# xiezheng-cs/PyTorch_Distributed_Template

Measured on AMD Instinct MI355X. Metric: images/sec (node) ResNet-18 DDP bs=1200/GPU at 1/2/4/8 MI355X, higher is better.
Workload: dtype bf16; 1 GPU; model=resnet18, global_batch=1200, parallelism=dp1, per_gpu_batch=1200, sync_bn=False, engine=native-hip, comm=none, grad_compress=none

## Files before the change

csrc/kernels/conv_fwd.h:

```cpp
#pragma once
#include <hip/hip_runtime.h>
#include <stdint.h>

#include "conv_geom.h"

namespace pdt {

constexpr int kStatSlots = 64;

void stat_rows_reduce_launch(const float* rows, int R, int CK, double* slots, hipStream_t s, int slots_ld = 0);


struct ConvFwdArgs : ConvGeom {
  const uint16_t* x;
  const uint16_t* w;
  uint16_t* y;
  const uint16_t* res;
  double* stats;
  int bnb;
  const uint16_t* bn_y1;
  const float* bn_coef1;
  const uint16_t* bn_y2;
  const float* bn_coef2;
  const uint8_t* bn_mask;
  int pair_skip;
  int res_phase = -1;
  int stage_out = 0;
  const float* pre_coef = nullptr;
  int ldy = 0, coef_ld = 0, stats_ld = 0;
  int nslice = 0;
  int64_t slice_wstride = 0;
  int srows_coff = 0;
};

void conv_fwd_launch(const ConvFwdArgs& a, int dtype, int bm, int bn, int bk, hipStream_t s);
int conv_fwd_m_tiles(int64_t M, int bm);

}
```

csrc/kernels/conv_fwd.hip:

```cpp
#include <cstdlib>

#include "../common.h"
#include "conv_fwd.h"
#include "conv_l1.h"

namespace pdt {

typedef __attribute__((address_space(3))) void lds_void;
typedef __attribute__((address_space(1))) void glb_void;

template <int CHUNKS>
PDT_DEVICE int swz(int row) { return (row >> 1) & (CHUNKS - 1); }

template <int DT, int EPI, int RES, int FN, int FM, int WN, int WM, int BN, int WAVES_M, int NW_, int SMEM = 0,
          bool PERM = false>
PDT_DEVICE void conv_epilogue(const ConvFwdArgs& a, f32x4_t (&acc)[FN][FM], int64_t m0, int n0, int tile_m, int wn,
                              int wm, int tid, int lane, char* smem) {
  using E = E16<DT>;
  const int fr = lane & 15, fq = lane >> 4;
  const int PQ = a.Pm * a.Qm;
  const FastDiv fd_pq{a.pq_mul, a.pq_shift}, fd_q{a.q_mul, a.q_shift};
  constexpr int KS = EPI == 0 ? 0 : (EPI == 4 ? 3 : 2);
  float sacc[FN][4][KS > 0 ? KS : 1];
#pragma unroll
  for (int i = 0; i < FN; ++i)
#pragma unroll
    for (int r = 0; r < 4; ++r)
#pragma unroll
      for (int k = 0; k < (KS > 0 ? KS : 1); ++k) sacc[i][r][k] = 0.f;

  constexpr int RED_BYTES = WAVES_M * BN * 3 * 4;
  float* cf = (float*)(smem + RED_BYTES);
  const int64_t LDY = a.ldy ? a.ldy : a.Kout;
  if constexpr (EPI >= 2) {
    const int CL = a.coef_ld ? a.coef_ld : a.Kout;
    for (int c = tid; c < BN; c += NW_ * 64) {
      const int n = n0 + c;
      cf[0 * BN + c] = a.bn_coef1[n];
      cf[1 * BN + c] = a.bn_coef1[CL + n];
      cf[2 * BN + c] = a.bn_coef1[2 * CL + n];
      cf[3 * BN + c] = a.bn_coef1[3 * CL + n];
      if constexpr (EPI == 4) {
        cf[4 * BN + c] = a.bn_coef2[2 * CL + n];
        cf[5 * BN + c] = a.bn_coef2[3 * CL + n];
      }
    }
    __syncthreads();
  }
  auto chan = [&](int i, int r) { return PERM ? (i >> 1) * 32 + 8 * fq + 4 * (i & 1) + r : i * 16 + 4 * fq + r; };
  static_assert(!PERM || FN % 2 == 0, "PERM pairs fragments");
  auto coef4 = [&](int q, int i) { return *(const float4*)(cf + q * BN + wn * WN + chan(i, 0)); };

  constexpr bool LY1 = EPI >= 2, LY2 = EPI == 4, LM = EPI == 3 || EPI == 4;
  static_assert(!LM || WN % 64 == 0, "bitmask epilogue needs 64-channel wave columns");
  constexpr int MW = LM ? WN / 64 : 1;
  constexpr int PER_J = FN * (2 * (RES != 0) + 2 * LY1 + 2 * LY2) + (LM ? 2 * MW : 0);
  constexpr int BUDGET = (FN * FM * 4 >= 128 ? 64 : 96) - (KS > 2 ? FN * 4 * (KS - 2) * 2 : 0);
  constexpr int JC = PER_J == 0 ? FM
                     : (8 * PER_J <= BUDGET && FM % 8 == 0) ? 8
                     : (4 * PER_J <= BUDGET && FM % 4 == 0) ? 4
                     : (2 * PER_J <= BUDGET && FM % 2 == 0) ? 2 : 1;
  static_assert(FM % JC == 0, "epilogue chunking");
  constexpr int BM_T = WAVES_M * WM;
  constexpr int SPITCH = BN * 2 + 16;
  constexpr int STG_OFF = 16384;
  constexpr bool FULL = SMEM >= STG_OFF + BM_T * SPITCH;
  constexpr bool PERGRP = !FULL && WAVES_M > 1 && EPI != 2 && SMEM >= STG_OFF + WM * SPITCH;
  constexpr bool CAN_STAGE = FULL || PERGRP;
  static_assert(!CAN_STAGE || RED_BYTES + 6 * BN * 4 <= STG_OFF, "epilogue LDS regions overlap");
  const bool stage = CAN_STAGE && a.stage_out;
  char* stg = smem + STG_OFF;
  const int srow0 = FULL ? wm * WM : 0;
  constexpr bool RC = RES == 2;
  const bool res_on = !RC || (int)blockIdx.y == a.res_phase;
  auto copy_rows = [&](int g) {
    constexpr int CPR = BN / 8;
    constexpr int SROWS = FULL ? BM_T : WM;
    for (int q = tid; q < SROWS * CPR; q += NW_ * 64) {
      const int row = q / CPR, ch = q - row * CPR;
      const int64_t m = m0 + (FULL ? 0 : g * WM) + row;
      if (m < a.M) {
        const int mm = (int)m;
        const int nimg = (int)fdiv((uint32_t)mm, fd_pq);
        const int rem = mm - nimg * PQ;
        const int i_ = (int)fdiv((uint32_t)rem, fd_q), j_ = rem - i_ * a.Qm;
        const int oh = i_ * a.ost_h + a.ooff_h, ow = j_ * a.ost_w + a.ooff_w;
        const int64_t ob = (((int64_t)nimg * a.OH + oh) * a.OW + ow) * LDY + n0 + ch * 8;
        *(uint4*)(a.y + ob) = *(const uint4*)(stg + row * SPITCH + ch * 16);
      }
    }
  };
  if constexpr (PERGRP) {
    if (stage)
      for (int g = 0; g < wm; ++g) {
        __syncthreads();
        copy_rows(g);
        __syncthreads();
      }
  }
#pragma unroll
  for (int jc = 0; jc < FM; jc += JC) {
    int64_t obase[JC];
    uint32_t rbase[RC ? JC : 1];
    bool valid[JC];
#pragma unroll
    for (int jj = 0; jj < JC; ++jj) {
      const int64_t m = m0 + wm * WM + (jc + jj) * 16 + fr;
      valid[jj] = m < a.M;
      const int mm = valid[jj] ? (int)m : 0;
      const int nimg = (int)fdiv((uint32_t)mm, fd_pq);
      const int rem = mm - nimg * PQ;
      const int i_ = (int)fdiv((uint32_t)rem, fd_q), j_ = rem - i_ * a.Qm;
      const int oh = i_ * a.ost_h + a.ooff_h, ow = j_ * a.ost_w + a.ooff_w;
      obase[jj] = (((int64_t)nimg * a.OH + oh) * a.OW + ow) * LDY;
      if constexpr (RC) rbase[jj] = (uint32_t)mm * (uint32_t)LDY;
    }
    uint2 p_res[RES ? JC : 1][RES ? FN : 1], p_y1[LY1 ? JC : 1][LY1 ? FN : 1], p_y2[LY2 ? JC : 1][LY2 ? FN : 1];
    uint64_t p_m[LM ? JC : 1][MW];
#pragma unroll
    for (int jj = 0; jj < JC; ++jj) {
      if constexpr (PERM) {
#pragma unroll
        for (int i = 0; i < FN; i += 2) {
          const int64_t o = obase[jj] + n0 + wn * WN + chan(i, 0);
          auto split = [&](uint2 (&dst)[FN], const uint4 v) {
            dst[i] = make_uint2(v.x, v.y);
            dst[i + 1] = make_uint2(v.z, v.w);
          };
          if constexpr (RES == 1) split(p_res[jj], *(const uint4*)(a.res + o));
          if constexpr (RC) split(p_res[jj], *(const uint4*)(a.res + rbase[jj] + (uint32_t)(n0 + wn * WN + chan(i, 0))));
          if constexpr (LY1) split(p_y1[jj], *(const uint4*)(a.bn_y1 + o));
          if constexpr (LY2) split(p_y2[jj], *(const uint4*)(a.bn_y2 + o));
        }
      } else {
#pragma unroll
        for (int i = 0; i < FN; ++i) {
          const int64_t o = obase[jj] + n0 + wn * WN + i * 16 + 4 * fq;
          if constexpr (RES == 1) p_res[jj][i] = *(const uint2*)(a.res + o);
          if constexpr (RC) p_res[jj][i] = *(const uint2*)(a.res + rbase[jj] + (uint32_t)(n0 + wn * WN + i * 16 + 4 * fq));
          if constexpr (LY1) p_y1[jj][i] = *(const uint2*)(a.bn_y1 + o);
          if constexpr (LY2) p_y2[jj][i] = *(const uint2*)(a.bn_y2 + o);
        }
      }
      if constexpr (LM) {
#pragma unroll
        for (int g = 0; g < MW; ++g)
          p_m[jj][g] = *(const uint64_t*)(a.bn_mask + ((obase[jj] + n0 + wn * WN + g * 64) >> 3));
      }
    }
#pragma unroll
    for (int jj = 0; jj < JC; ++jj) {
      if (!valid[jj]) continue;
      const int j = jc + jj;
      uint2 held = make_uint2(0u, 0u);
#pragma unroll
      for (int i = 0; i < FN; ++i) {
        const int n = n0 + wn * WN + chan(i, 0);
        const int64_t o = obase[jj] + n;
        float v[4] = {acc[i][j][0], acc[i][j][1], acc[i][j][2], acc[i][j][3]};
        if constexpr (RES) {
          uint2 rr = p_res[jj][i];
          if constexpr (RC) {
            rr.x = res_on ? rr.x : 0u;
            rr.y = res_on ? rr.y : 0u;
          }
          v[0] += E::to_f((uint16_t)(rr.x & 0xffff));
          v[1] += E::to_f((uint16_t)(rr.x >> 16));
          v[2] += E::to_f((uint16_t)(rr.y & 0xffff));
          v[3] += E::to_f((uint16_t)(rr.y >> 16));
        }
        float y1[4], y2[4];
        if constexpr (LY1) {
          const uint2 q1 = p_y1[jj][i];
          y1[0] = E::to_f((uint16_t)(q1.x & 0xffff)); y1[1] = E::to_f((uint16_t)(q1.x >> 16));
          y1[2] = E::to_f((uint16_t)(q1.y & 0xffff)); y1[3] = E::to_f((uint16_t)(q1.y >> 16));
          if constexpr (EPI == 2) {
            const float4 sc = coef4(0, i), sh = coef4(1, i);
            if (!(y1[0] * sc.x + sh.x > 0.f)) v[0] = 0.f;
            if (!(y1[1] * sc.y + sh.y > 0.f)) v[1] = 0.f;
            if (!(y1[2] * sc.z + sh.z > 0.f)) v[2] = 0.f;
            if (!(y1[3] * sc.w + sh.w > 0.f)) v[3] = 0.f;
          } else {
            const uint32_t mb = (uint32_t)(p_m[jj][chan(i, 0) >> 6] >> (chan(i, 0) & 63));
            if (!(mb & 1u)) v[0] = 0.f;
            if (!(mb & 2u)) v[1] = 0.f;
            if (!(mb & 4u)) v[2] = 0.f;
            if (!(mb & 8u)) v[3] = 0.f;
          }
        }
        if constexpr (LY2) {
          const uint2 q2 = p_y2[jj][i];
          y2[0] = E::to_f((uint16_t)(q2.x & 0xffff)); y2[1] = E::to_f((uint16_t)(q2.x >> 16));
          y2[2] = E::to_f((uint16_t)(q2.y & 0xffff)); y2[3] = E::to_f((uint16_t)(q2.y >> 16));
        }
        uint2 packed;
        packed.x = E::pack2(v[0], v[1]);
        packed.y = E::pack2(v[2], v[3]);
        const uint16_t ov[4] = {(uint16_t)packed.x, (uint16_t)(packed.x >> 16), (uint16_t)packed.y,
                                (uint16_t)(packed.y >> 16)};
        if (CAN_STAGE && stage) {
          if constexpr (PERM) {
            if (i & 1)
              *(uint4*)(stg + (srow0 + j * 16 + fr) * SPITCH + (wn * WN + chan(i, 0) - 4) * 2) =
                  make_uint4(held.x, held.y, packed.x, packed.y);
            else
              held = packed;
          } else {
            *(uint2*)(stg + (srow0 + j * 16 + fr) * SPITCH + (wn * WN + chan(i, 0)) * 2) = packed;
          }
        } else if constexpr (PERM) {
          if (i & 1)
            *(uint4*)(a.y + o - 4) = make_uint4(held.x, held.y, packed.x, packed.y);
          else
            held = packed;
        } else {
          *(uint2*)(a.y + o) = packed;
        }
        if constexpr (EPI == 1) {
#pragma unroll
          for (int r = 0; r < 4; ++r) {
            const float q = E::to_f(ov[r]);
            sacc[i][r][0] += q;
            sacc[i][r][1] += q * q;
          }
        } else if constexpr (EPI >= 2) {
          const float4 mu = coef4(2, i), is = coef4(3, i);
          const float m1[4] = {mu.x, mu.y, mu.z, mu.w}, i1[4] = {is.x, is.y, is.z, is.w};
#pragma unroll
          for (int r = 0; r < 4; ++r) {
            const float dz = E::to_f(ov[r]);
            sacc[i][r][0] += dz;
            sacc[i][r][1] += dz * (y1[r] - m1[r]) * i1[r];
          }
          if constexpr (EPI == 4) {
            const float4 mu2 = coef4(4, i), is2 = coef4(5, i);
            const float m2[4] = {mu2.x, mu2.y, mu2.z, mu2.w}, i2[4] = {is2.x, is2.y, is2.z, is2.w};
#pragma unroll
            for (int r = 0; r < 4; ++r) sacc[i][r][2] += E::to_f(ov[r]) * (y2[r] - m2[r]) * i2[r];
          }
        }
      }
    }
  }

  if constexpr (CAN_STAGE) {
    if (stage) {
      if constexpr (PERGRP) {
        for (int g = wm; g < WAVES_M; ++g) {
          __syncthreads();
          copy_rows(g);
          __syncthreads();
        }
      } else {
        __syncthreads();
        copy_rows(0);
      }
    }
  }

  if constexpr (KS > 0) {
    constexpr int KO = EPI == 4 ? 4 : 2;
#pragma unroll
    for (int i = 0; i < FN; ++i)
#pragma unroll
      for (int r = 0; r < 4; ++r)
#pragma unroll
        for (int k = 0; k < KS; ++k) sacc[i][r][k] = row16_sum(sacc[i][r][k]);
    float* red = (float*)smem;
    __syncthreads();
    if (fr == 15) {
#pragma unroll
      for (int i = 0; i < FN; ++i)
#pragma unroll
        for (int r = 0; r < 4; ++r) {
          const int nl = wn * WN + chan(i, r);
#pragma unroll
          for (int k = 0; k < KS; ++k) red[(wm * BN + nl) * KS + k] = sacc[i][r][k];
        }
    }
    __syncthreads();
    if (tid < BN) {
      float t[KS];
#pragma unroll
      for (int k = 0; k < KS; ++k) t[k] = 0.f;
#pragma unroll
      for (int w = 0; w < WAVES_M; ++w)
#pragma unroll
        for (int k = 0; k < KS; ++k) t[k] += red[(w * BN + tid) * KS + k];
      const int64_t row = (a.nphase > 0 ? (int64_t)blockIdx.y * a.srows_pp : 0) + tile_m;
// ... 21 lines not shown
template <int DT, int BM, int BN, int BK, int WAVES_N, int EPI, int RES, int STAGES, int NW>
__global__ __launch_bounds__(NW * 64, (STAGES * (BN + BM) * BK * 2 <= 81920 || NW == 8) ? 2 : 1)
void conv_fwd_kernel(ConvFwdArgs args) {
  ConvFwdArgs a = args;
  const uint16_t* wbase = args.w;
  if (args.nslice > 1) {
    const int sl = blockIdx.z;
    a.x += (int64_t)sl * a.Kout;
    a.y += (int64_t)sl * a.Kout;
    wbase += (int64_t)sl * args.slice_wstride;
    a.w = wbase;
    if (a.bn_y1 != nullptr) a.bn_y1 += (int64_t)sl * a.Kout;
    if (a.bn_coef1 != nullptr) a.bn_coef1 += sl * a.Kout;
    a.srows_coff = sl * a.Kout;
  }
  if (args.nphase > 0 && !select_phase(a, args, wbase, blockIdx.y)) {
    zero_stat_row<EPI, BN>(a, NW * 64);
    return;
  }
  using E = E16<DT>;
  typedef typename E::vec8 vec8;
  constexpr int WAVES_M = NW / WAVES_N;
  constexpr int WN = BN / WAVES_N;
  constexpr int WM = BM / WAVES_M;
  constexpr int FN = WN / 16, FM = WM / 16;
  constexpr int ROWB = BK * 2;
  constexpr int CHUNKS = ROWB / 16;
  constexpr int RPI = 1024 / ROWB;
  constexpr int A_INSTR = BN / RPI / NW;
  constexpr int B_INSTR = BM / RPI / NW;
  constexpr int A_BYTES = BN * ROWB;
  constexpr int STAGE = (BN + BM) * ROWB;
  static_assert(A_INSTR * RPI * NW == BN && B_INSTR * RPI * NW == BM, "tile/instr mismatch");
  __shared__ __attribute__((aligned(1024))) char smem[STAGES * STAGE];

  const int tid = threadIdx.x;
  const int lane = tid & 63;
  const int wave = __builtin_amdgcn_readfirstlane(tid >> 6);
  const int wn = wave % WAVES_N, wm = wave / WAVES_N;

  const int nwg = a.m_tiles * a.n_tiles;
  const int bid = xcd_remap(blockIdx.x, nwg);
  const int tile_m = bid / a.n_tiles, tile_n = bid % a.n_tiles;
  const int64_t m0 = (int64_t)tile_m * BM;
  const int n0 = tile_n * BN;

  const int PQ = a.Pm * a.Qm;
  const FastDiv fd_pq{a.pq_mul, a.pq_shift}, fd_q{a.q_mul, a.q_shift};
  const int TU = a.T * a.U;
  const int csteps = a.C / BK;
  const int ksteps = TU * csteps;

  const __amdgpu_buffer_rsrc_t rx = make_rsrc(a.x, (uint32_t)a.N * a.H * a.W * a.cs * 2u);
  const __amdgpu_buffer_rsrc_t rw = make_rsrc(a.w, (uint32_t)a.Kout * TU * a.C * 2u);

  const int lrow = lane / CHUNKS;
  const int pchunk = lane % CHUNKS;
  int brow_h[B_INSTR], brow_w[B_INSTR], brow_off[B_INSTR];
#pragma unroll
  for (int j = 0; j < B_INSTR; ++j) {
    const int row = (wave * B_INSTR + j) * RPI + lrow;
    const int64_t m = m0 + row;
    const int bch = pchunk ^ swz<CHUNKS>(row);
    if (m < a.M) {
      const int nimg = (int)fdiv((uint32_t)m, fd_pq);
      const int rem = (int)m - nimg * PQ;
      const int i = (int)fdiv((uint32_t)rem, fd_q), jj = rem - i * a.Qm;
      brow_h[j] = i * a.ist_h + a.ioff_h;
      brow_w[j] = jj * a.ist_w + a.ioff_w;
      const int pair = (CHUNKS == 8 && bch >= 4) ? a.pair_skip : 0;
      brow_off[j] = (((nimg * a.H + brow_h[j]) * a.W + brow_w[j]) * a.cs + bch * 8 + pair) * 2;
    } else {
      brow_h[j] = -(1 << 29);
      brow_w[j] = 0;
      brow_off[j] = 0;
    }
  }
  constexpr bool PERM = WN % 32 == 0;
  uint32_t arow_off[A_INSTR];
#pragma unroll
  for (int j = 0; j < A_INSTR; ++j) {
    const int row = (wave * A_INSTR + j) * RPI + lrow;
    const int lw = row % WN, fi = lw >> 4, fm = lw & 15;
    const int ch = PERM ? row - lw + (fi >> 1) * 32 + (fm >> 2) * 8 + (fi & 1) * 4 + (fm & 3) : row;
// ... 33 lines not shown
  const int fr = lane & 15, fq = lane >> 4;
  int a_off[FN], b_off[FM];
#pragma unroll
  for (int i = 0; i < FN; ++i) a_off[i] = (wn * WN + i * 16 + fr) * ROWB;
#pragma unroll
  for (int j = 0; j < FM; ++j) b_off[j] = A_BYTES + (wm * WM + j * 16 + fr) * ROWB;

  auto compute_stage = [&](const char* sb) {
#pragma unroll
    for (int kk = 0; kk < BK / 32; ++kk) {
      vec8 af[FN], bfr[FM];
#pragma unroll
      for (int i = 0; i < FN; ++i) {
        const int row = wn * WN + i * 16 + fr;
        const int ch = (kk * 4 + fq) ^ swz<CHUNKS>(row);
        af[i] = *(const vec8*)(sb + a_off[i] + ch * 16);
      }
#pragma unroll
      for (int j = 0; j < FM; ++j) {
        const int row = wm * WM + j * 16 + fr;
        const int ch = (kk * 4 + fq) ^ swz<CHUNKS>(row);
        bfr[j] = *(const vec8*)(sb + b_off[j] + ch * 16);
      }
#pragma unroll
      for (int i = 0; i < FN; ++i)
#pragma unroll
        for (int j = 0; j < FM; ++j) acc[i][j] = E::mfma16x16x32(af[i], bfr[j], acc[i][j]);
    }
  };

  if constexpr (STAGES == 2) {
    if (ksteps > 0) {
      stage_load(0);
      asm volatile("s_waitcnt vmcnt(0)" ::: "memory");
      __syncthreads();
      for (int ks = 0; ks < ksteps; ++ks) {
        const int cur = ks & 1;
        if (ks + 1 < ksteps) stage_load(cur ^ 1);
        compute_stage(smem + cur * STAGE);
        asm volatile("s_waitcnt vmcnt(0)" ::: "memory");
        __syncthreads();
      }
    }
  } else {
    constexpr int S = STAGES;
    constexpr int PER_STAGE = A_INSTR + B_INSTR;
    auto wait_ahead = [&](int ahead) {
      constexpr int W1 = PER_STAGE, W2 = 2 * PER_STAGE;
      if (ahead >= 2)
        __builtin_amdgcn_s_waitcnt((W2 & 0xF) | ((W2 >> 4) << 14) | (0x7 << 4) | (0xF << 8));
      else if (ahead == 1)
        __builtin_amdgcn_s_waitcnt((W1 & 0xF) | ((W1 >> 4) << 14) | (0x7 << 4) | (0xF << 8));
      else
        asm volatile("s_waitcnt vmcnt(0)" ::: "memory");
    };
    static_assert(S <= 4, "wait_ahead covers at most two stages in flight");
    if (ksteps > 0) {
#pragma unroll
      for (int p = 0; p < S - 1; ++p)
        if (p < ksteps) stage_load(p);
      int buf = 0;
      for (int ks = 0; ks < ksteps; ++ks) {
        const int ahead = min(S - 2, ksteps - 1 - ks);
        wait_ahead(ahead);
        __builtin_amdgcn_s_barrier();
        if (ks + S - 1 < ksteps) stage_load(buf == 0 ? S - 1 : buf - 1);
        __builtin_amdgcn_s_setprio(1);
        compute_stage(smem + buf * STAGE);
        __builtin_amdgcn_s_setprio(0);
        buf = buf == S - 1 ? 0 : buf + 1;
      }
      asm volatile("s_waitcnt lgkmcnt(0)" ::: "memory");
      __builtin_amdgcn_s_barrier();
    }
  }

  conv_epilogue<DT, EPI, RES, FN, FM, WN, WM, BN, WAVES_M, NW, STAGES * STAGE, PERM>(a, acc, m0, n0, tile_m, wn, wm, tid,
                                                                             lane, smem);
}

template <int N>
PDT_DEVICE void vm_wait() {
  static_assert(N >= 0 && N < 64, "vmcnt range");
  __builtin_amdgcn_s_waitcnt((N & 0xF) | ((N >> 4) << 14) | (0x7 << 4) | (0xF << 8));
}

template <int DT, int BM, int BN, int EPI, int RES, bool PP_STAGE = (EPI != 2)>
__global__ __launch_bounds__(512) void conv_pp_kernel(ConvFwdArgs args) {
  ConvFwdArgs a = args;
  if (args.nphase > 0 && !select_phase(a, args, args.w, blockIdx.y)) {
    zero_stat_row<EPI, BN>(a, 512);
    return;
  }
  using E = E16<DT>;
  typedef typename E::vec8 vec8;
  constexpr int NW = 8, WN = 64, WM = 128;
  constexpr int WAVES_N = BN / WN, WAVES_M = NW / WAVES_N;
  static_assert(WAVES_N * WAVES_M == NW && WAVES_M * WM == BM, "pp tile geometry");
  constexpr int FN = 4, FM = 8;
  constexpr int ROWB = 128;
  constexpr int XH = (BM / 2) * ROWB;
  constexpr int WH = (BN / 2) * ROWB;
  constexpr int NX = XH / 1024 / NW;
  constexpr int NWI = WH / 1024 / NW;
  static_assert(NX * 1024 * NW == XH && NWI * 1024 * NW == WH, "pp DMA split");
  constexpr int BUF = 2 * XH + 2 * WH;
  constexpr int OX0 = 0, OX1 = XH, OW0 = 2 * XH, OW1 = 2 * XH + WH;
  __shared__ __attribute__((aligned(1024))) char smem[2 * BUF];

  const int tid = threadIdx.x;
  const int lane = tid & 63;
  const int wave = __builtin_amdgcn_readfirstlane(tid >> 6);
  const int grp = wave >> 2;
  const int wn = wave % WAVES_N, wm = wave / WAVES_N;

  const int nwg = a.m_tiles * a.n_tiles;
  const int bid = xcd_remap(blockIdx.x, nwg);
  const int tile_m = bid / a.n_tiles, tile_n = bid % a.n_tiles;
  const int64_t m0 = (int64_t)tile_m * BM;
  const int n0 = tile_n * BN;

  const int PQ = a.Pm * a.Qm;
  const FastDiv fd_pq{a.pq_mul, a.pq_shift}, fd_q{a.q_mul, a.q_shift};
  const int TU = a.T * a.U;
  const int csteps = a.C >> 6;
  const int ksteps = TU * csteps;

  const __amdgpu_buffer_rsrc_t rx = make_rsrc(a.x, (uint32_t)a.N * a.H * a.W * a.cs * 2u);
  const __amdgpu_buffer_rsrc_t rw = make_rsrc(a.w, (uint32_t)a.Kout * TU * a.C * 2u);

  const int lrow = lane >> 3, pchunk = lane & 7;
  int xhw[2][NX], xoff[2][NX];
#pragma unroll
  for (int h = 0; h < 2; ++h)
#pragma unroll
    for (int j = 0; j < NX; ++j) {
      const int hr = (wave * NX + j) * 8 + lrow;
      const int64_t m = m0 + (hr >> 6) * 128 + h * 64 + (hr & 63);
      const int bch = pchunk ^ ((hr >> 1) & 7);
      if (m < a.M) {
        const int nimg = (int)fdiv((uint32_t)m, fd_pq);
        const int rem = (int)m - nimg * PQ;
        const int i = (int)fdiv((uint32_t)rem, fd_q), jj = rem - i * a.Qm;
        const int ih = i * a.ist_h + a.ioff_h, iw = jj * a.ist_w + a.ioff_w;
        xhw[h][j] = (ih << 16) | (iw & 0xffff);
        xoff[h][j] = (((nimg * a.H + ih) * a.W + iw) * a.cs + bch * 8) * 2;
      } else {
        xhw[h][j] = (int)0xC0000000;
        xoff[h][j] = 0;
      }
    }
  uint32_t woff[2][NWI];
#pragma unroll
  for (int h = 0; h < 2; ++h)
#pragma unroll
    for (int j = 0; j < NWI; ++j) {
      const int hr = (wave * NWI + j) * 8 + lrow;
      const int lr = hr & 31;
      const int n = n0 + (hr >> 5) * 64 + h * 32 + ((lr & 15) >> 2) * 8 + (lr >> 4) * 4 + (lr & 3);
// ... 49 lines not shown
#pragma unroll
    for (int f = 0; f < 2; ++f)
#pragma unroll
      for (int kk = 0; kk < 2; ++kk)
        wr[f][kk] = *(const vec8*)(base + (wrow0 + f * 16) * ROWB + (((kk * 4 + fq) ^ sw) << 4));
  };
  auto mma = [&](const vec8 (&wr)[2][2], int xh, int wh) {
#pragma unroll
    for (int kk = 0; kk < 2; ++kk)
#pragma unroll
      for (int f2 = 0; f2 < 2; ++f2)
#pragma unroll
        for (int f = 0; f < 4; ++f)
          acc[wh * 2 + f2][xh * 4 + f] = E::mfma16x16x32(wr[f2][kk], xs[f][kk], acc[wh * 2 + f2][xh * 4 + f]);
  };
  auto compute = [&](const vec8 (&wr)[2][2], int xh, int wh) {
    __builtin_amdgcn_sched_barrier(0);
    __builtin_amdgcn_s_barrier();
    __builtin_amdgcn_sched_barrier(0);
    __builtin_amdgcn_s_setprio(1);
    mma(wr, xh, wh);
    __builtin_amdgcn_s_setprio(0);
    __builtin_amdgcn_sched_barrier(0);
    __builtin_amdgcn_s_barrier();
    __builtin_amdgcn_sched_barrier(0);
  };

  if (ksteps > 0) {
    advance();
    dma_x(smem, 0);
    dma_w(smem, 0);
    dma_w(smem, 1);
    dma_x(smem, 1);
    vm_wait<NWI + NX>();
    __builtin_amdgcn_sched_barrier(0);
    __builtin_amdgcn_s_barrier();
    if (grp == 1) __builtin_amdgcn_s_barrier();
    for (int ks = 0; ks < ksteps; ++ks) {
      const char* cb = smem + (ks & 1) * BUF;
      char* nb = smem + ((ks + 1) & 1) * BUF;
      const bool more = ks + 1 < ksteps;
      if (more) advance();
      if (more) { dma_x(nb, 0); vm_wait<2 * NX>(); } else { vm_wait<NX>(); }
      read_x(cb + OX0);
      read_w(w0r, cb + OW0);
      compute(w0r, 0, 0);
      if (more) { dma_w(nb, 0); vm_wait<NX + NWI>(); } else { vm_wait<0>(); }
      read_w(w1r, cb + OW1);
      compute(w1r, 0, 1);
      if (more) dma_w(nb, 1);
      read_x(cb + OX1);
      compute(w1r, 1, 1);
      if (more) { dma_x(nb, 1); vm_wait<NWI + NX>(); }
      compute(w0r, 1, 0);
    }
    if (grp == 0) __builtin_amdgcn_s_barrier();
    asm volatile("s_waitcnt vmcnt(0) lgkmcnt(0)" ::: "memory");
    __builtin_amdgcn_s_barrier();
  }

  conv_epilogue<DT, EPI, RES, FN, FM, WN, WM, BN, WAVES_M, NW, PP_STAGE ? 2 * BUF : 0, true>(a, acc, m0, n0, tile_m, wn,
                                                                                        wm, tid, lane, smem);
}

template <int DT, int BM, int BN>
static void launch_pp(const ConvFwdArgs& args, int gx, hipStream_t s) {
  ConvFwdArgs a = args;
  a.stage_out = 0;
  if (a.nslice > 1)
    pdt_hip_fail("conv_pp: slice-batched (grouped) launches run on the generic kernel", hipErrorInvalidValue, __FILE__,
                 __LINE__);
  dim3 grid(gx, a.nphase > 0 ? a.nphase : 1), block(512);
  const int rs = a.res == nullptr ? 0 : (a.res_phase >= 0 && a.nphase > 0 ? 2 : 1);
  const int epi = a.bnb ? a.bnb + 1 : (a.stats != nullptr ? 1 : 0);
#define PDT_K(E_, R_) hipLaunchKernelGGL((conv_pp_kernel<DT, BM, BN, E_, R_>), grid, block, 0, s, a)
  if (epi == 0) {
    if (rs == 1) PDT_K(0, 1); else if (rs == 2) PDT_K(0, 2); else PDT_K(0, 0);
  } else if (epi == 1 && rs != 2) {
    if (rs) PDT_K(1, 1); else PDT_K(1, 0);
  } else if (epi == 2 && !rs) {
    PDT_K(2, 0);
  } else if (epi == 3 && rs) {
    if (rs == 2) PDT_K(3, 2); else PDT_K(3, 1);
  } else if (epi == 4 && rs) {
    if (rs == 2) PDT_K(4, 2); else PDT_K(4, 1);
  } else {
    pdt_hip_fail("conv_pp: unsupported epilogue variant", hipErrorInvalidValue, __FILE__, __LINE__);
  }
#undef PDT_K
}

template <int DT, int BM, int BN, int BK, int WAVES_N, int STAGES, int NW>
static void launch_cfg(const ConvFwdArgs& a, int gx, hipStream_t s) {
  dim3 grid(gx, a.nphase > 0 ? a.nphase : 1, a.nslice > 1 ? a.nslice : 1), block(NW * 64);
  const int rs = a.res == nullptr ? 0 : (a.res_phase >= 0 && a.nphase > 0 ? 2 : 1);
  const int epi = a.bnb ? a.bnb + 1 : (a.stats != nullptr ? 1 : 0);
#define PDT_K(E_, R_) hipLaunchKernelGGL((conv_fwd_kernel<DT, BM, BN, BK, WAVES_N, E_, R_, STAGES, NW>), grid, block, 0, s, a)
  if (epi == 0) {
    if (rs == 1) PDT_K(0, 1); else if (rs == 2) PDT_K(0, 2); else PDT_K(0, 0);
  } else if (epi == 1 && rs != 2) {
    if (rs) PDT_K(1, 1); else PDT_K(1, 0);
  } else if constexpr ((((BK == 64 && STAGES == 2) || (BK == 32 && STAGES == 3)) && (BN == 128 || BN == 64) &&
                        (BM * BN == 4096 * NW || (BM == 256 && BN == 128 && NW == 4))) ||
                       (BM == 256 && BN == 256)) {
    if (epi == 2 && !rs) PDT_K(2, 0);
    else if (epi == 3 && rs) { if (rs == 2) PDT_K(3, 2); else PDT_K(3, 1); }
    else if (epi == 4 && rs) { if (rs == 2) PDT_K(4, 2); else PDT_K(4, 1); }
    else pdt_hip_fail("conv_fwd: unsupported BN-backward epilogue variant", hipErrorInvalidValue, __FILE__, __LINE__);
  } else {
    pdt_hip_fail("conv_fwd: BN-backward epilogue needs a 128x128 or 256x64 tile", hipErrorInvalidValue,
                 __FILE__, __LINE__);
  }
#undef PDT_K
}

template <int DT>
static void launch_tile(const ConvFwdArgs& a, int gx, int bm, int bn, int bk, hipStream_t s);

template <int DT>
static void launch_dt(ConvFwdArgs a, int bm, int bn, int bk, hipStream_t s) {
  a.stage_out = 0;
  int gx = 0;
  const int srows = conv_geom_plan(a, bm, bn, &gx);
  if (gx == 0) return;
  const int KO = a.bnb == 3 ? 4 : 2;
  const int nsl = a.nslice > 1 ? a.nslice : 1;
  Scratch part(a.stats ? (size_t)srows * a.Kout * nsl * KO * sizeof(float) : 0, s);
  a.srows = part.as<float>();
  launch_tile<DT>(a, gx, bm, bn, bk, s);
  if (a.stats) stat_rows_reduce_launch(a.srows, srows, a.Kout * nsl * KO, a.stats, s, a.stats_ld);
}

template <int DT>
static void launch_tile(const ConvFwdArgs& a, int gx, int bm, int bn, int bk, hipStream_t s) {
#define PDT_CFGN(BM_, BN_, BK_, WN_, ST_, NW_)            \
  if (bm == BM_ && bn == BN_ && bk == BK_) {               \
    launch_cfg<DT, BM_, BN_, BK_, WN_, ST_, NW_>(a, gx, s); \
    return;                                                \
  }
#define PDT_CFG(BM_, BN_, BK_, WN_, ST_) PDT_CFGN(BM_, BN_, BK_, WN_, ST_, 4)
  {
    const bool dg = a.nphase > 0;
    const bool pp = bk == 64 && a.C % 64 == 0 && ((bm == 256 && bn == 256) || (bm == 512 && bn == 128));
    if (pp && dg)
      PDT_COUNT("conv_pp_dgrad");
    else if (pp)
      PDT_COUNT("conv_pp_fwd");
    else if (dg && a.nphase > 1)
      PDT_COUNT("conv_generic_dgrad_phased");
    else if (dg)
      PDT_COUNT("conv_generic_dgrad");
    else if (a.cs != a.C)
      PDT_COUNT("conv_generic_fwd_window");
    else
// ... 79 lines not shown
```

Before: 63210 images/s.

## Software-pipeline BN-backward epilogue loads and prestage BN coefficients during mainloop

For the BN-backward epilogues (EPI>=2), the y1/y2/residual/mask loads are now issued as asm global loads several fragment rows ahead, with explicit vmcnt waits, instead of being loaded in chunks and then consumed. The BN coefficient table is moved into an extra LDS region that is filled during the conv prologue when LDS allows, which removes a __syncthreads at the start of the epilogue. The unused staged-output path is dropped. The trade-off is more LDS per block and higher register pressure from the prefetched sets, which could lower occupancy.

```diff
diff --git a/csrc/kernels/conv_fwd.h b/csrc/kernels/conv_fwd.h
--- a/csrc/kernels/conv_fwd.h
+++ b/csrc/kernels/conv_fwd.h
@@ -25,7 +25,6 @@
   const uint8_t* bn_mask;
   int pair_skip;
   int res_phase = -1;
-  int stage_out = 0;
   const float* pre_coef = nullptr;
   int ldy = 0, coef_ld = 0, stats_ld = 0;
   int nslice = 0;
diff --git a/csrc/kernels/conv_fwd.hip b/csrc/kernels/conv_fwd.hip
--- a/csrc/kernels/conv_fwd.hip
+++ b/csrc/kernels/conv_fwd.hip
@@ -1,4 +1,5 @@
 #include <cstdlib>
+#include <type_traits>
 
 #include "../common.h"
 #include "conv_fwd.h"
@@ -12,10 +13,40 @@
 template <int CHUNKS>
 PDT_DEVICE int swz(int row) { return (row >> 1) & (CHUNKS - 1); }
 
-template <int DT, int EPI, int RES, int FN, int FM, int WN, int WM, int BN, int WAVES_M, int NW_, int SMEM = 0,
-          bool PERM = false>
+template <int EPI, int BN, int NT>
+PDT_DEVICE void stage_bn_coef(const ConvFwdArgs& a, float* cf, int n0, int tid) {
+  const int CL = a.coef_ld ? a.coef_ld : a.Kout;
+  for (int c = tid; c < BN; c += NT) {
+    const int n = n0 + c;
+    cf[0 * BN + c] = a.bn_coef1[n];
+    cf[1 * BN + c] = a.bn_coef1[CL + n];
+    cf[2 * BN + c] = a.bn_coef1[2 * CL + n];
+    cf[3 * BN + c] = a.bn_coef1[3 * CL + n];
+    if constexpr (EPI == 4) {
+      cf[4 * BN + c] = a.bn_coef2[2 * CL + n];
+      cf[5 * BN + c] = a.bn_coef2[3 * CL + n];
+    }
+  }
+}
+
+template <int I, int N, class F>
+PDT_DEVICE void static_for(F&& f) {
+  if constexpr (I < N) {
+    f(std::integral_constant<int, I>{});
+    static_for<I + 1, N>(f);
+  }
+}
+
+template <int N>
+PDT_DEVICE void vm_wait_asm() {
+  static_assert(N >= 0 && N < 64, "vmcnt range");
+  asm volatile("s_waitcnt vmcnt(%0)" : : "n"(N) : "memory");
+}
+
+template <int DT, int EPI, int RES, int FN, int FM, int WN, int WM, int BN, int WAVES_M, int NW_, bool PERM = false,
+          bool CF_PRE = false>
 PDT_DEVICE void conv_epilogue(const ConvFwdArgs& a, f32x4_t (&acc)[FN][FM], int64_t m0, int n0, int tile_m, int wn,
-                              int wm, int tid, int lane, char* smem) {
+                              int wm, int tid, int lane, char* smem, float* cf_pre = nullptr) {
   using E = E16<DT>;
   const int fr = lane & 15, fq = lane >> 4;
   const int PQ = a.Pm * a.Qm;
@@ -30,28 +61,15 @@
       for (int k = 0; k < (KS > 0 ? KS : 1); ++k) sacc[i][r][k] = 0.f;
 
   constexpr int RED_BYTES = WAVES_M * BN * 3 * 4;
-  float* cf = (float*)(smem + RED_BYTES);
+  float* cf = CF_PRE ? cf_pre : (float*)(smem + RED_BYTES);
   const int64_t LDY = a.ldy ? a.ldy : a.Kout;
-  if constexpr (EPI >= 2) {
-    const int CL = a.coef_ld ? a.coef_ld : a.Kout;
-    for (int c = tid; c < BN; c += NW_ * 64) {
-      const int n = n0 + c;
-      cf[0 * BN + c] = a.bn_coef1[n];
-      cf[1 * BN + c] = a.bn_coef1[CL + n];
-      cf[2 * BN + c] = a.bn_coef1[2 * CL + n];
-      cf[3 * BN + c] = a.bn_coef1[3 * CL + n];
-      if constexpr (EPI == 4) {
-        cf[4 * BN + c] = a.bn_coef2[2 * CL + n];
-        cf[5 * BN + c] = a.bn_coef2[3 * CL + n];
-      }
-    }
-    __syncthreads();
-  }
+  static_assert(EPI < 2 || PERM, "the BN-backward epilogues run on 64-channel wave columns (fragment pairs)");
   auto chan = [&](int i, int r) { return PERM ? (i >> 1) * 32 + 8 * fq + 4 * (i & 1) + r : i * 16 + 4 * fq + r; };
   static_assert(!PERM || FN % 2 == 0, "PERM pairs fragments");
   auto coef4 = [&](int q, int i) { return *(const float4*)(cf + q * BN + wn * WN + chan(i, 0)); };
 
   constexpr bool LY1 = EPI >= 2, LY2 = EPI == 4, LM = EPI == 3 || EPI == 4;
+  constexpr bool PIPE = EPI >= 2;
   static_assert(!LM || WN % 64 == 0, "bitmask epilogue needs 64-channel wave columns");
   constexpr int MW = LM ? WN / 64 : 1;
   constexpr int PER_J = FN * (2 * (RES != 0) + 2 * LY1 + 2 * LY2) + (LM ? 2 * MW : 0);
@@ -61,200 +79,203 @@
                      : (4 * PER_J <= BUDGET && FM % 4 == 0) ? 4
                      : (2 * PER_J <= BUDGET && FM % 2 == 0) ? 2 : 1;
   static_assert(FM % JC == 0, "epilogue chunking");
-  constexpr int BM_T = WAVES_M * WM;
-  constexpr int SPITCH = BN * 2 + 16;
-  constexpr int STG_OFF = 16384;
-  constexpr bool FULL = SMEM >= STG_OFF + BM_T * SPITCH;
-  constexpr bool PERGRP = !FULL && WAVES_M > 1 && EPI != 2 && SMEM >= STG_OFF + WM * SPITCH;
-  constexpr bool CAN_STAGE = FULL || PERGRP;
-  static_assert(!CAN_STAGE || RED_BYTES + 6 * BN * 4 <= STG_OFF, "epilogue LDS regions overlap");
-  const bool stage = CAN_STAGE && a.stage_out;
-  char* stg = smem + STG_OFF;
-  const int srow0 = FULL ? wm * WM : 0;
+  constexpr int NP = FN / 2;
+  constexpr int NLJ = NP * ((RES != 0) + LY1 + LY2) + (LM ? MW : 0);
+  constexpr int PBUDGET = (FN * FM * 4 >= 128 ? 56 : 96) - (KS > 2 ? FN * 4 * (KS - 2) : 0) - (EPI == 2 ? 8 : 0);
+  constexpr int PSETS = !PIPE ? 1 : PBUDGET / PER_J < 1 ? 1 : PBUDGET / PER_J > FM ? FM : PBUDGET / PER_J;
+  constexpr int PD = PSETS - 1;
+  static_assert(PD * NLJ < 64, "vmcnt range");
   constexpr bool RC = RES == 2;
   const bool res_on = !RC || (int)blockIdx.y == a.res_phase;
-  auto copy_rows = [&](int g) {
-    constexpr int CPR = BN / 8;
-    constexpr int SROWS = FULL ? BM_T : WM;
-    for (int q = tid; q < SROWS * CPR; q += NW_ * 64) {
-      const int row = q / CPR, ch = q - row * CPR;
-      const int64_t m = m0 + (FULL ? 0 : g * WM) + row;
-      if (m < a.M) {
-        const int mm = (int)m;
-        const int nimg = (int)fdiv((uint32_t)mm, fd_pq);
-        const int rem = mm - nimg * PQ;
-        const int i_ = (int)fdiv((uint32_t)rem, fd_q), j_ = rem - i_ * a.Qm;
-        const int oh = i_ * a.ost_h + a.ooff_h, ow = j_ * a.ost_w + a.ooff_w;
-        const int64_t ob = (((int64_t)nimg * a.OH + oh) * a.OW + ow) * LDY + n0 + ch * 8;
-        *(uint4*)(a.y + ob) = *(const uint4*)(stg + row * SPITCH + ch * 16);
-      }
-    }
-  };
-  if constexpr (PERGRP) {
-    if (stage)
-      for (int g = 0; g < wm; ++g) {
-        __syncthreads();
-        copy_rows(g);
-        __syncthreads();
-      }
-  }
-#pragma unroll
-  for (int jc = 0; jc < FM; jc += JC) {
-    int64_t obase[JC];
-    uint32_t rbase[RC ? JC : 1];
-    bool valid[JC];
-#pragma unroll
-    for (int jj = 0; jj < JC; ++jj) {
-      const int64_t m = m0 + wm * WM + (jc + jj) * 16 + fr;
-      valid[jj] = m < a.M;
-      const int mm = valid[jj] ? (int)m : 0;
-      const int nimg = (int)fdiv((uint32_t)mm, fd_pq);
-      const int rem = mm - nimg * PQ;
-      const int i_ = (int)fdiv((uint32_t)rem, fd_q), j_ = rem - i_ * a.Qm;
-      const int oh = i_ * a.ost_h + a.ooff_h, ow = j_ * a.ost_w + a.ooff_w;
-      obase[jj] = (((int64_t)nimg * a.OH + oh) * a.OW + ow) * LDY;
-      if constexpr (RC) rbase[jj] = (uint32_t)mm * (uint32_t)LDY;
-    }
-    uint2 p_res[RES ? JC : 1][RES ? FN : 1], p_y1[LY1 ? JC : 1][LY1 ? FN : 1], p_y2[LY2 ? JC : 1][LY2 ? FN : 1];
-    uint64_t p_m[LM ? JC : 1][MW];
-#pragma unroll
-    for (int jj = 0; jj < JC; ++jj) {
+  auto pixel = [&](int j, bool& valid, uint32_t& rbase) -> int64_t {
+    const int64_t m = m0 + wm * WM + j * 16 + fr;
+    valid = m < a.M;
+    const int mm = valid ? (int)m : 0;
+    const int nimg = (int)fdiv((uint32_t)mm, fd_pq);
+    const int rem = mm - nimg * PQ;
+    const int i_ = (int)fdiv((uint32_t)rem, fd_q), j_ = rem - i_ * a.Qm;
+    const int oh = i_ * a.ost_h + a.ooff_h, ow = j_ * a.ost_w + a.ooff_w;
+    rbase = (uint32_t)mm * (uint32_t)LDY;
+    return (((int64_t)nimg * a.OH + oh) * a.OW + ow) * LDY;
+  };
+  auto frag = [&](int j, int64_t ob, const uint2 (&pr)[RES ? FN : 1], const uint2 (&py1)[LY1 ? FN : 1],
+                  const uint2 (&py2)[LY2 ? FN : 1], const uint64_t (&pm)[MW]) {
+    uint2 held = make_uint2(0u, 0u);
+#pragma unroll
+    for (int i = 0; i < FN; ++i) {
+      const int n = n0 + wn * WN + chan(i, 0);
+      const int64_t o = ob + n;
+      float v[4] = {acc[i][j][0], acc[i][j][1], acc[i][j][2], acc[i][j][3]};
+      if constexpr (RES) {
+        uint2 rr = pr[i];
+        if constexpr (RC) {
+          rr.x = res_on ? rr.x : 0u;
+          rr.y = res_on ? rr.y : 0u;
+        }
+        v[0] += E::to_f((uint16_t)(rr.x & 0xffff));
+        v[1] += E::to_f((uint16_t)(rr.x >> 16));
+        v[2] += E::to_f((uint16_t)(rr.y & 0xffff));
+        v[3] += E::to_f((uint16_t)(rr.y >> 16));
+      }
+      float y1[4], y2[4];
+      if constexpr (LY1) {
+        const uint2 q1 = py1[i];
+        y1[0] = E::to_f((uint16_t)(q1.x & 0xffff)); y1[1] = E::to_f((uint16_t)(q1.x >> 16));
+        y1[2] = E::to_f((uint16_t)(q1.y & 0xffff)); y1[3] = E::to_f((uint16_t)(q1.y >> 16));
+        if constexpr (EPI == 2) {
+          const float4 sc = coef4(0, i), sh = coef4(1, i);
+          if (!(y1[0] * sc.x + sh.x > 0.f)) v[0] = 0.f;
+          if (!(y1[1] * sc.y + sh.y > 0.f)) v[1] = 0.f;
+          if (!(y1[2] * sc.z + sh.z > 0.f)) v[2] = 0.f;
+          if (!(y1[3] * sc.w + sh.w > 0.f)) v[3] = 0.f;
+        } else {
+          const uint32_t mb = (uint32_t)(pm[chan(i, 0) >> 6] >> (chan(i, 0) & 63));
+          if (!(mb & 1u)) v[0] = 0.f;
+          if (!(mb & 2u)) v[1] = 0.f;
+          if (!(mb & 4u)) v[2] = 0.f;
+          if (!(mb & 8u)) v[3] = 0.f;
+        }
+      }
+      if constexpr (LY2) {
+        const uint2 q2 = py2[i];
+        y2[0] = E::to_f((uint16_t)(q2.x & 0xffff)); y2[1] = E::to_f((uint16_t)(q2.x >> 16));
+        y2[2] = E::to_f((uint16_t)(q2.y & 0xffff)); y2[3] = E::to_f((uint16_t)(q2.y >> 16));
+      }
+      uint2 packed;
+      packed.x = E::pack2(v[0], v[1]);
+      packed.y = E::pack2(v[2], v[3]);
+      const uint16_t ov[4] = {(uint16_t)packed.x, (uint16_t)(packed.x >> 16), (uint16_t)packed.y,
+                              (uint16_t)(packed.y >> 16)};
       if constexpr (PERM) {
-#pragma unroll
-        for (int i = 0; i < FN; i += 2) {
-          const int64_t o = obase[jj] + n0 + wn * WN + chan(i, 0);
-          auto split = [&](uint2 (&dst)[FN], const uint4 v) {
-            dst[i] = make_uint2(v.x, v.y);
-            dst[i + 1] = make_uint2(v.z, v.w);
-          };
-          if constexpr (RES == 1) split(p_res[jj], *(const uint4*)(a.res + o));
-          if constexpr (RC) split(p_res[jj], *(const uint4*)(a.res + rbase[jj] + (uint32_t)(n0 + wn * WN + chan(i, 0))));
-          if constexpr (LY1) split(p_y1[jj], *(const uint4*)(a.bn_y1 + o));
-          if constexpr (LY2) split(p_y2[jj], *(const uint4*)(a.bn_y2 + o));
+        if (i & 1)
+          *(uint4*)(a.y + o - 4) = make_uint4(held.x, held.y, packed.x, packed.y);
+        else
+          held = packed;
+      } else {
+        *(uint2*)(a.y + o) = packed;
+      }
+      if constexpr (EPI == 1) {
+#pragma unroll
+        for (int r = 0; r < 4; ++r) {
+          const float q = E::to_f(ov[r]);
+          sacc[i][r][0] += q;
+          sacc[i][r][1] += q * q;
         }
-      } else {
-#pragma unroll
-        for (int i = 0; i < FN; ++i) {
-          const int64_t o = obase[jj] + n0 + wn * WN + i * 16 + 4 * fq;
-          if constexpr (RES == 1) p_res[jj][i] = *(const uint2*)(a.res + o);
-          if constexpr (RC) p_res[jj][i] = *(const uint2*)(a.res + rbase[jj] + (uint32_t)(n0 + wn * WN + i * 16 + 4 * fq));
-          if constexpr (LY1) p_y1[jj][i] = *(const uint2*)(a.bn_y1 + o);
-          if constexpr (LY2) p_y2[jj][i] = *(const uint2*)(a.bn_y2 + o);
+      } else if constexpr (EPI >= 2) {
+        const float4 mu = coef4(2, i), is = coef4(3, i);
+        const float m1[4] = {mu.x, mu.y, mu.z, mu.w}, i1[4] = {is.x, is.y, is.z, is.w};
+#pragma unroll
+        for (int r = 0; r < 4; ++r) {
+          const float dz = E::to_f(ov[r]);
+          sacc[i][r][0] += dz;
+          sacc[i][r][1] += dz * (y1[r] - m1[r]) * i1[r];
         }
+        if constexpr (EPI == 4) {
+          const float4 mu2 = coef4(4, i), is2 = coef4(5, i);
+          const float m2[4] = {mu2.x, mu2.y, mu2.z, mu2.w}, i2[4] = {is2.x, is2.y, is2.z, is2.w};
+#pragma unroll
+          for (int r = 0; r < 4; ++r) sacc[i][r][2] += E::to_f(ov[r]) * (y2[r] - m2[r]) * i2[r];
+        }
+      }
+    }
+  };
+
+  if constexpr (PIPE) {
+    u32x4v q_res[RES ? FM : 1][NP], q_y1[FM][NP], q_y2[LY2 ? FM : 1][NP];
+    u32x2v q_m[LM ? FM : 1][MW];
+    int64_t obase[FM];
+    auto issue = [&](int j) {
+      bool valid;
+      uint32_t rbase;
+      obase[j] = pixel(j, valid, rbase);
+#pragma unroll
+      for (int p = 0; p < NP; ++p) {
+        const int c = n0 + wn * WN + chan(2 * p, 0);
+        if constexpr (RES == 1) q_res[j][p] = gload16_asm(a.res + obase[j] + c);
+        if constexpr (RC) q_res[j][p] = gload16_asm(a.res + rbase + (uint32_t)c);
+        q_y1[j][p] = gload16_asm(a.bn_y1 + obase[j] + c);
+        if constexpr (LY2) q_y2[j][p] = gload16_asm(a.bn_y2 + obase[j] + c);
       }
       if constexpr (LM) {
 #pragma unroll
-        for (int g = 0; g < MW; ++g)
-          p_m[jj][g] = *(const uint64_t*)(a.bn_mask + ((obase[jj] + n0 + wn * WN + g * 64) >> 3));
-      }
-    }
-#pragma unroll
-    for (int jj = 0; jj < JC; ++jj) {
-      if (!valid[jj]) continue;
-      const int j = jc + jj;
-      uint2 held = make_uint2(0u, 0u);
-#pragma unroll
-      for (int i = 0; i < FN; ++i) {
-        const int n = n0 + wn * WN + chan(i, 0);
-        const int64_t o = obase[jj] + n;
-        float v[4] = {acc[i][j][0], acc[i][j][1], acc[i][j][2], acc[i][j][3]};
-        if constexpr (RES) {
-          uint2 rr = p_res[jj][i];
-          if constexpr (RC) {
-            rr.x = res_on ? rr.x : 0u;
-            rr.y = res_on ? rr.y : 0u;
+        for (int g = 0; g < MW; ++g) q_m[j][g] = gload8_asm(a.bn_mask + ((obase[j] + n0 + wn * WN + g * 64) >> 3));
+      }
+    };
+#pragma unroll
+    for (int j = 0; j < PD; ++j) issue(j);
+    if constexpr (!CF_PRE) {
+      stage_bn_coef<EPI, BN, NW_ * 64>(a, cf, n0, tid);
+      __syncthreads();
+    }
+    static_for<0, FM>([&](auto J) {
+      constexpr int j = decltype(J)::value;
+      if constexpr (j + PD < FM) issue(j + PD);
+      vm_wait_asm<(FM - 1 - j < PD ? FM - 1 - j : PD) * NLJ>();
+      uint2 pr[RES ? FN : 1], py1[FN], py2[LY2 ? FN : 1];
+      uint64_t pm[MW];
+#pragma unroll
+      for (int p = 0; p < NP; ++p) {
+        asm volatile("" : "+v"(q_y1[j][p]));
+        py1[2 * p] = make_uint2(q_y1[j][p][0], q_y1[j][p][1]);
+        py1[2 * p + 1] = make_uint2(q_y1[j][p][2], q_y1[j][p][3]);
+        if constexpr (RES != 0) {
+          asm volatile("" : "+v"(q_res[j][p]));
+          pr[2 * p] = make_uint2(q_res[j][p][0], q_res[j][p][1]);
+          pr[2 * p + 1] = make_uint2(q_res[j][p][2], q_res[j][p][3]);
+        }
+        if constexpr (LY2) {
+          asm volatile("" : "+v"(q_y2[j][p]));
+          py2[2 * p] = make_uint2(q_y2[j][p][0], q_y2[j][p][1]);
+          py2[2 * p + 1] = make_uint2(q_y2[j][p][2], q_y2[j][p][3]);
+        }
+      }
+#pragma unroll
+      for (int g = 0; g < MW; ++g) {
+        if constexpr (LM) {
+          asm volatile("" : "+v"(q_m[j][g]));
+          pm[g] = (uint64_t)q_m[j][g][0] | ((uint64_t)q_m[j][g][1] << 32);
+        } else {
+          pm[g] = 0;
+        }
+      }
+      if (m0 + wm * WM + j * 16 + fr < a.M) frag(j, obase[j], pr, py1, py2, pm);
+    });
+  } else {
+#pragma unroll
+    for (int jc = 0; jc < FM; jc += JC) {
+      int64_t obase[JC];
+      uint32_t rbase[RC ? JC : 1];
+      bool valid[JC];
+      uint2 p_res[RES ? JC : 1][RES ? FN : 1], p_y1[1][1], p_y2[1][1];
+      uint64_t p_m[1][MW];
+#pragma unroll
+      for (int jj = 0; jj < JC; ++jj) {
+        uint32_t rb;
+        obase[jj] = pixel(jc + jj, valid[jj], rb);
+        if constexpr (RC) rbase[jj] = rb;
+        if constexpr (PERM) {
+#pragma unroll
+          for (int i = 0; i < FN; i += 2) {
+            const int64_t o = obase[jj] + n0 + wn * WN + chan(i, 0);
+            auto split = [&](uint2 (&dst)[FN], const uint4 v) {
+              dst[i] = make_uint2(v.x, v.y);
+              dst[i + 1] = make_uint2(v.z, v.w);
+            };
+            if constexpr (RES == 1) split(p_res[jj], *(const uint4*)(a.res + o));
+            if constexpr (RC) split(p_res[jj], *(const uint4*)(a.res + rbase[jj] + (uint32_t)(n0 + wn * WN + chan(i, 0))));
           }
-          v[0] += E::to_f((uint16_t)(rr.x & 0xffff));
-          v[1] += E::to_f((uint16_t)(rr.x >> 16));
-          v[2] += E::to_f((uint16_t)(rr.y & 0xffff));
-          v[3] += E::to_f((uint16_t)(rr.y >> 16));
-        }
-        float y1[4], y2[4];
-        if constexpr (LY1) {
-          const uint2 q1 = p_y1[jj][i];
-          y1[0] = E::to_f((uint16_t)(q1.x & 0xffff)); y1[1] = E::to_f((uint16_t)(q1.x >> 16));
-          y1[2] = E::to_f((uint16_t)(q1.y & 0xffff)); y1[3] = E::to_f((uint16_t)(q1.y >> 16));
-          if constexpr (EPI == 2) {
-            const float4 sc = coef4(0, i), sh = coef4(1, i);
-            if (!(y1[0] * sc.x + sh.x > 0.f)) v[0] = 0.f;
-            if (!(y1[1] * sc.y + sh.y > 0.f)) v[1] = 0.f;
-            if (!(y1[2] * sc.z + sh.z > 0.f)) v[2] = 0.f;
-            if (!(y1[3] * sc.w + sh.w > 0.f)) v[3] = 0.f;
-          } else {
-            const uint32_t mb = (uint32_t)(p_m[jj][chan(i, 0) >> 6] >> (chan(i, 0) & 63));
-            if (!(mb & 1u)) v[0] = 0.f;
-            if (!(mb & 2u)) v[1] = 0.f;
-            if (!(mb & 4u)) v[2] = 0.f;
-            if (!(mb & 8u)) v[3] = 0.f;
+        } else {
+#pragma unroll
+          for (int i = 0; i < FN; ++i) {
+            const int64_t o = obase[jj] + n0 + wn * WN + i * 16 + 4 * fq;
+            if constexpr (RES == 1) p_res[jj][i] = *(const uint2*)(a.res + o);
+            if constexpr (RC) p_res[jj][i] = *(const uint2*)(a.res + rbase[jj] + (uint32_t)(n0 + wn * WN + i * 16 + 4 * fq));
           }
         }
-        if constexpr (LY2) {
-          const uint2 q2 = p_y2[jj][i];
-          y2[0] = E::to_f((uint16_t)(q2.x & 0xffff)); y2[1] = E::to_f((uint16_t)(q2.x >> 16));
-          y2[2] = E::to_f((uint16_t)(q2.y & 0xffff)); y2[3] = E::to_f((uint16_t)(q2.y >> 16));
-        }
-        uint2 packed;
-        packed.x = E::pack2(v[0], v[1]);
-        packed.y = E::pack2(v[2], v[3]);
-        const uint16_t ov[4] = {(uint16_t)packed.x, (uint16_t)(packed.x >> 16), (uint16_t)packed.y,
-                                (uint16_t)(packed.y >> 16)};
-        if (CAN_STAGE && stage) {
-          if constexpr (PERM) {
-            if (i & 1)
-              *(uint4*)(stg + (srow0 + j * 16 + fr) * SPITCH + (wn * WN + chan(i, 0) - 4) * 2) =
-                  make_uint4(held.x, held.y, packed.x, packed.y);
-            else
-              held = packed;
-          } else {
-            *(uint2*)(stg + (srow0 + j * 16 + fr) * SPITCH + (wn * WN + chan(i, 0)) * 2) = packed;
-          }
-        } else if constexpr (PERM) {
-          if (i & 1)
-            *(uint4*)(a.y + o - 4) = make_uint4(held.x, held.y, packed.x, packed.y);
-          else
-            held = packed;
-        } else {
-          *(uint2*)(a.y + o) = packed;
-        }
-        if constexpr (EPI == 1) {
-#pragma unroll
-          for (int r = 0; r < 4; ++r) {
-            const float q = E::to_f(ov[r]);
-            sacc[i][r][0] += q;
-            sacc[i][r][1] += q * q;
-          }
-        } else if constexpr (EPI >= 2) {
-          const float4 mu = coef4(2, i), is = coef4(3, i);
-          const float m1[4] = {mu.x, mu.y, mu.z, mu.w}, i1[4] = {is.x, is.y, is.z, is.w};
-#pragma unroll
-          for (int r = 0; r < 4; ++r) {
-            const float dz = E::to_f(ov[r]);
-            sacc[i][r][0] += dz;
-            sacc[i][r][1] += dz * (y1[r] - m1[r]) * i1[r];
-          }
-          if constexpr (EPI == 4) {
-            const float4 mu2 = coef4(4, i), is2 = coef4(5, i);
-            const float m2[4] = {mu2.x, mu2.y, mu2.z, mu2.w}, i2[4] = {is2.x, is2.y, is2.z, is2.w};
-#pragma unroll
-            for (int r = 0; r < 4; ++r) sacc[i][r][2] += E::to_f(ov[r]) * (y2[r] - m2[r]) * i2[r];
-          }
-        }
-      }
-    }
-  }
-
-  if constexpr (CAN_STAGE) {
-    if (stage) {
-      if constexpr (PERGRP) {
-        for (int g = wm; g < WAVES_M; ++g) {
-          __syncthreads();
-          copy_rows(g);
-          __syncthreads();
-        }
-      } else {
-        __syncthreads();
-        copy_rows(0);
-      }
+      }
+#pragma unroll
+      for (int jj = 0; jj < JC; ++jj)
+        if (valid[jj]) frag(jc + jj, obase[jj], p_res[jj], p_y1[0], p_y2[0], p_m[0]);
     }
   }
 
@@ -342,7 +363,9 @@
   constexpr int A_BYTES = BN * ROWB;
   constexpr int STAGE = (BN + BM) * ROWB;
   static_assert(A_INSTR * RPI * NW == BN && B_INSTR * RPI * NW == BM, "tile/instr mismatch");
-  __shared__ __attribute__((aligned(1024))) char smem[STAGES * STAGE];
+  constexpr int RING = STAGES * STAGE, CF_BYTES = 6 * BN * 4;
+  constexpr bool CF_PRE = EPI >= 2 && STAGES == 2 && RING + CF_BYTES <= 81920;
+  __shared__ __attribute__((aligned(1024))) char smem[RING + (CF_PRE ? CF_BYTES : 0)];
 
   const int tid = threadIdx.x;
   const int lane = tid & 63;
@@ -360,6 +383,9 @@
   const int TU = a.T * a.U;
   const int csteps = a.C / BK;
   const int ksteps = TU * csteps;
+  auto stage_cf = [&]() {
+    if constexpr (CF_PRE) stage_bn_coef<EPI, BN, NW * 64>(a, (float*)(smem + RING), n0, tid);
+  };
 
   const __amdgpu_buffer_rsrc_t rx = make_rsrc(a.x, (uint32_t)a.N * a.H * a.W * a.cs * 2u);
   const __amdgpu_buffer_rsrc_t rw = make_rsrc(a.w, (uint32_t)a.Kout * TU * a.C * 2u);
@@ -459,6 +485,7 @@
   if constexpr (STAGES == 2) {
     if (ksteps > 0) {
       stage_load(0);
+      stage_cf();
       asm volatile("s_waitcnt vmcnt(0)" ::: "memory");
       __syncthreads();
       for (int ks = 0; ks < ksteps; ++ks) {
@@ -468,6 +495,9 @@
         asm volatile("s_waitcnt vmcnt(0)" ::: "memory");
         __syncthreads();
       }
+    } else if constexpr (CF_PRE) {
+      stage_cf();
+      __syncthreads();
     }
   } else {
     constexpr int S = STAGES;
@@ -502,8 +532,8 @@
     }
   }
 
-  conv_epilogue<DT, EPI, RES, FN, FM, WN, WM, BN, WAVES_M, NW, STAGES * STAGE, PERM>(a, acc, m0, n0, tile_m, wn, wm, tid,
-                                                                             lane, smem);
+  conv_epilogue<DT, EPI, RES, FN, FM, WN, WM, BN, WAVES_M, NW, PERM, CF_PRE>(a, acc, m0, n0, tile_m, wn, wm, tid, lane,
+                                                                            smem, (float*)(smem + RING));
 }
 
 template <int N>
@@ -512,7 +542,7 @@
   __builtin_amdgcn_s_waitcnt((N & 0xF) | ((N >> 4) << 14) | (0x7 << 4) | (0xF << 8));
 }
 
-template <int DT, int BM, int BN, int EPI, int RES, bool PP_STAGE = (EPI != 2)>
+template <int DT, int BM, int BN, int EPI, int RES>
 __global__ __launch_bounds__(512) void conv_pp_kernel(ConvFwdArgs args) {
   ConvFwdArgs a = args;
   if (args.nphase > 0 && !select_phase(a, args, args.w, blockIdx.y)) {
@@ -533,7 +563,9 @@
   static_assert(NX * 1024 * NW == XH && NWI * 1024 * NW == WH, "pp DMA split");
   constexpr int BUF = 2 * XH + 2 * WH;
   constexpr int OX0 = 0, OX1 = XH, OW0 = 2 * XH, OW1 = 2 * XH + WH;
-  __shared__ __attribute__((aligned(1024))) char smem[2 * BUF];
+  constexpr int CF_BYTES = 6 * BN * 4;
+  constexpr bool CF_PRE = EPI >= 2 && 2 * BUF + CF_BYTES <= 163840;
+  __shared__ __attribute__((aligned(1024))) char smem[2 * BUF + (CF_PRE ? CF_BYTES : 0)];
 
   const int tid = threadIdx.x;
   const int lane = tid & 63;
@@ -552,6 +584,9 @@
   const int TU = a.T * a.U;
   const int csteps = a.C >> 6;
   const int ksteps = TU * csteps;
+  auto stage_cf = [&]() {
+    if constexpr (CF_PRE) stage_bn_coef<EPI, BN, 512>(a, (float*)(smem + 2 * BUF), n0, tid);
+  };
 
   const __amdgpu_buffer_rsrc_t rx = make_rsrc(a.x, (uint32_t)a.N * a.H * a.W * a.cs * 2u);
   const __amdgpu_buffer_rsrc_t rw = make_rsrc(a.w, (uint32_t)a.Kout * TU * a.C * 2u);
@@ -667,6 +702,7 @@
     dma_w(smem, 0);
     dma_w(smem, 1);
     dma_x(smem, 1);
+    stage_cf();
     vm_wait<NWI + NX>();
     __builtin_amdgcn_sched_barrier(0);
     __builtin_amdgcn_s_barrier();
@@ -692,16 +728,18 @@
     if (grp == 0) __builtin_amdgcn_s_barrier();
     asm volatile("s_waitcnt vmcnt(0) lgkmcnt(0)" ::: "memory");
     __builtin_amdgcn_s_barrier();
-  }
-
-  conv_epilogue<DT, EPI, RES, FN, FM, WN, WM, BN, WAVES_M, NW, PP_STAGE ? 2 * BUF : 0, true>(a, acc, m0, n0, tile_m, wn,
-                                                                                        wm, tid, lane, smem);
+  } else if constexpr (CF_PRE) {
+    stage_cf();
+    __syncthreads();
+  }
+
+  conv_epilogue<DT, EPI, RES, FN, FM, WN, WM, BN, WAVES_M, NW, true, CF_PRE>(
+      a, acc, m0, n0, tile_m, wn, wm, tid, lane, smem, (float*)(smem + 2 * BUF));
 }
 
 template <int DT, int BM, int BN>
 static void launch_pp(const ConvFwdArgs& args, int gx, hipStream_t s) {
   ConvFwdArgs a = args;
-  a.stage_out = 0;
   if (a.nslice > 1)
     pdt_hip_fail("conv_pp: slice-batched (grouped) launches run on the generic kernel", hipErrorInvalidValue, __FILE__,
                  __LINE__);
@@ -754,7 +792,6 @@
 
 template <int DT>
 static void launch_dt(ConvFwdArgs a, int bm, int bn, int bk, hipStream_t s) {
-  a.stage_out = 0;
   int gx = 0;
   const int srows = conv_geom_plan(a, bm, bn, &gx);
   if (gx == 0) return;
```

Measured after the change: 63650 images/s (median of 6 runs). No clear change (+0.7%).
